# arun-sub/genomicsbench

Measured on AMD Instinct MI355X. Metric: bsw_large_gcups, higher is better.
Workload: dtype int32

## Files before the change

genomicsbench_amd/csrc/bsw_kernels.hip:

```cpp
#include "gbx_internal.h"
#include <atomic>
#include <climits>
#include <cstdlib>

namespace gbx {
namespace {

constexpr int NEG = -(1 << 29);
constexpr int BIGJ = 1 << 20;

constexpr int NCLS = 21;
constexpr int CLS_LDS = NCLS - 1;
constexpr int NTB = 32;
constexpr int NBIN = NCLS * NTB;
constexpr int HDR = 1024;
constexpr int REG_SCORE_LIMIT = 1 << 20;

struct BswDev {
    int o_del, e_del, o_ins, e_ins, oe_del, oe_ins, zdrop, end_bonus, w, max_mat;
    uint32_t colword[5];
    int32_t col4[5];
    uint32_t row0[5];
    uint32_t row1[5];
    uint8_t remap[24];
    uint32_t lrow[5];
    int lane_on;
};

struct BswPairs {
    const uint8_t *ref, *qer;
    const int64_t *idr, *idq;
    const int32_t *len1, *len2, *h0;
    gbx_bsw_result *out;
    int packed = 0;
};

constexpr int WS_HDR = 4 * HDR;
struct BswWork {
    int32_t *counts, *cursors, *base, *bad, *order, *wband;
    int32_t *lbase, *lrank, *lorder, *lchunk;
};

__host__ __device__ inline int cls_of(int qlen, int bound)
{
    if (qlen > 1024 || bound >= REG_SCORE_LIMIT) return CLS_LDS;
    if (qlen > 256) return 19;
    if (qlen <= 128) return (qlen - 1) >> 3;
    return qlen <= 160 ? 16 : qlen <= 192 ? 17 : 18;
}
constexpr int LANE_QMAX = 159;
constexpr int LANE_ROWS = 2 * (LANE_QMAX + 1);
constexpr int LANE_BINS = LANE_ROWS * 256;
constexpr int LANE_SCORE_LIMIT = 8192;
constexpr int LANE_COMPACT_LIMIT = 256;
constexpr int LANE_NRANGE = 5;
constexpr int LANE_RANGE_HI[2][LANE_NRANGE] = {{47, 79, 99, 135, LANE_QMAX}, {39, 79, 103, 127, LANE_QMAX}};
__host__ __device__ inline bool lane_ok(int lane_on, int qlen, int tlen, int h0, int max_mat)
{
    return lane_on && qlen >= 1 && qlen <= LANE_QMAX && tlen >= 1 && h0 >= 0 && h0 + qlen * (max_mat > 0 ? max_mat : 0) < LANE_SCORE_LIMIT;
}
__host__ __device__ inline int lane_key(int qlen, int h0, int max_mat)
{
    const int wide = h0 + qlen * (max_mat > 0 ? max_mat : 0) < LANE_COMPACT_LIMIT ? 0 : 1;
    return ((wide * (LANE_QMAX + 1) + qlen) << 8) | (h0 < 255 ? h0 : 255);
}

__host__ __device__ inline int bin_of(int cls, int tlen)
{
    const int tb = tlen >> 4;
    return cls * NTB + (NTB - 1 - (tb < NTB - 1 ? tb : NTB - 1));
}

__device__ inline int imax3(int a, int b, int c) { return max(max(a, b), c); }

template <int CTRL, int ROWMASK = 0xf, int BANKMASK = 0xf>
__device__ inline int dpp(int old, int x)
{
    return __builtin_amdgcn_update_dpp(old, x, CTRL, ROWMASK, BANKMASK, false);
}
// ... 479 lines not shown
            "v_max3_u32 %[key], %[kin], %[ka], %[kb]\n"
            "v_lshl_or_b32 %[wn], %[v], 16, %[u]\n"
            : [sa] "=&v"(sa), [ta] "=&v"(ta), [tb] "=&v"(tb), [ma] "=&v"(ma), [mb] "=&v"(mb), [x] "=&v"(x), [ha] "=&v"(ha),
              [hb] "=&v"(hb), [td] "=&v"(td), [ed] "=&v"(ed), [ena] "=&v"(ena), [enb] "=&v"(enb), [fd] "=&v"(fd), [ka] "=&v"(ka),
              [kb] "=&v"(kb), [u] "=&v"(u), [v] "=&v"(v), [wn] "=&v"(wn), [f] "+v"(f), [key] "=v"(kout)
            : [w] "v"(w), [qq] "v"(qq), [rw] "v"(rw), [rwn] "v"(rwn), [left] "v"(left), [kin] "v"(kin), [pa] "v"(pa), [pa1] "v"(pa1), [zero] "v"(zero), [oed] "s"(oe_del),
              [edel] "s"(e_del), [eins] "s"(e_ins)
            : "vcc");
    } else {
        int sa, ta, tb, ma, mb, x, ha, td, ti, ed, ena, enb, fd, ka, kb, u, v;
        asm volatile(
            "v_perm_b32 %[sa], %[rwn], %[rw], %[qq]\n"
            "v_cmp_ne_u32_sdwa vcc, %[w], %[zero] src0_sel:BYTE_1 src1_sel:DWORD\n"
            "v_subrev_u32 %[fd], %[eins], %[f]\n"
            "v_add_u32_sdwa %[ta], sext(%[sa]), %[w] dst_sel:DWORD dst_unused:UNUSED_PAD src0_sel:BYTE_0 src1_sel:BYTE_1\n"
            "v_cndmask_b32 %[ma], 0, %[ta], vcc\n"
            "v_cmp_ne_u32_sdwa vcc, %[w], %[zero] src0_sel:BYTE_3 src1_sel:DWORD\n"
            "v_max_i32_sdwa %[x], %[ma], %[w] dst_sel:DWORD dst_unused:UNUSED_PAD src0_sel:DWORD src1_sel:BYTE_0\n"
            "v_add_u32_sdwa %[tb], sext(%[sa]), %[w] dst_sel:DWORD dst_unused:UNUSED_PAD src0_sel:BYTE_1 src1_sel:BYTE_3\n"
            "v_max_i32 %[ha], %[x], %[f]\n"
            "v_subrev_u32 %[td], %[oed], %[ma]\n"
            "v_subrev_u32 %[ti], %[oei], %[ma]\n"
            "v_cndmask_b32 %[mb], 0, %[tb], vcc\n"
            "v_sub_u32_sdwa %[ed], %[w], %[edel] dst_sel:DWORD dst_unused:UNUSED_PAD src0_sel:BYTE_0 src1_sel:DWORD\n"
            "v_max3_i32 %[f], %[fd], %[ti], 0\n"
            "v_max3_i32 %[ena], %[ed], %[td], 0\n"
            "v_max_i32_sdwa %[x], %[mb], %[w] dst_sel:DWORD dst_unused:UNUSED_PAD src0_sel:DWORD src1_sel:BYTE_2\n"
            "v_lshl_or_b32 %[ka], %[ha], 18, %[pa]\n"
            "v_max_i32 %[hb], %[x], %[f]\n"
            "v_subrev_u32 %[td], %[oed], %[mb]\n"
            "v_subrev_u32 %[ti], %[oei], %[mb]\n"
            "v_subrev_u32 %[fd], %[eins], %[f]\n"
            "v_sub_u32_sdwa %[ed], %[w], %[edel] dst_sel:DWORD dst_unused:UNUSED_PAD src0_sel:BYTE_2 src1_sel:DWORD\n"
            "v_max3_i32 %[f], %[fd], %[ti], 0\n"
            "v_max3_i32 %[enb], %[ed], %[td], 0\n"
            "v_lshl_or_b32 %[kb], %[hb], 18, %[pa1]\n"
            "v_lshl_or_b32 %[u], %[left], 8, %[ena]\n"
            "v_lshl_or_b32 %[v], %[ha], 8, %[enb]\n"
            "v_max3_u32 %[key], %[kin], %[ka], %[kb]\n"
            "v_lshl_or_b32 %[wn], %[v], 16, %[u]\n"
            : [sa] "=&v"(sa), [ta] "=&v"(ta), [tb] "=&v"(tb), [ma] "=&v"(ma), [mb] "=&v"(mb), [x] "=&v"(x), [ha] "=&v"(ha),
              [hb] "=&v"(hb), [td] "=&v"(td), [ti] "=&v"(ti), [ed] "=&v"(ed), [ena] "=&v"(ena), [enb] "=&v"(enb), [fd] "=&v"(fd), [ka] "=&v"(ka),
              [kb] "=&v"(kb), [u] "=&v"(u), [v] "=&v"(v), [wn] "=&v"(wn), [f] "+v"(f), [key] "=v"(kout)
            : [w] "v"(w), [qq] "v"(qq), [rw] "v"(rw), [rwn] "v"(rwn), [left] "v"(left), [kin] "v"(kin), [pa] "v"(pa), [pa1] "v"(pa1), [zero] "v"(zero), [oed] "s"(oe_del),
              [oei] "s"(oe_ins), [edel] "s"(e_del), [eins] "s"(e_ins)
            : "vcc");
    }
    left = hb;
    key = kout;
    return wn;
}

#ifdef GBX_BSW_LANE_STATS
__device__ unsigned long long g_bsw_lane_stats[16][4];
#endif
template <bool SYM, bool COMPACT, bool CODE4 = false, bool PACKED = false>
__global__ void __launch_bounds__(64) bsw_lane_kernel(BswDev prm, BswPairs P, BswWork W, int rlo, int rhi, int cols, int slot)
{
    extern __shared__ uint32_t lcell[];
#ifdef GBX_BSW_LANE_STATS
    __shared__ int st_rowmax[2048];
    for (int k = threadIdx.x; k < 2048; k += 64) st_rowmax[k] = 0;
    unsigned long long st_cells = 0, st_rows = 0, st_wcells = 0, st_wrows = 0;
#endif
#define LCELL(byte_addr) (*(uint32_t *)((char *)lcell + (byte_addr)))
#define LCELL16(byte_addr) (*(uint16_t *)((char *)lcell + (byte_addr)))
#define LQ8(byte_addr) (*((uint8_t *)lcell + (byte_addr)))
    const int lane = threadIdx.x;
    const int first = W.lbase[rlo << 8], count = W.lbase[(rhi + 1) << 8] - first;
    const int nchunks = (count + 63) >> 6;
    const int32_t *order = W.lorder + first;
    const int e_ins = prm.e_ins, e_del = prm.e_del, oe_ins = prm.oe_ins, oe_del = prm.oe_del;
    const int cb = lane * 4;
    constexpr int QROW = CODE4 ? 64 : 128;
    const int qb = (cols >> 1) * 256 + (CODE4 ? lane : (lane & 31) * 4 + (lane >> 5) * 2);
    auto LQREAD = [&](int a) -> uint32_t { return CODE4 ? (uint32_t)LQ8(a) : (uint32_t)LCELL16(a); };
    auto QSEL = [](uint32_t q) -> uint32_t { return CODE4 ? (((q >> 4) << 8) | (q & 15u)) : q; };
    auto QLOW = [](uint32_t q) -> uint32_t { return CODE4 ? (q & 15u) : (q & 0xffu); };
    auto cell_at = [&](int j) { return COMPACT ? (j >> 1) * 256 + cb + (j & 1) * 2 : j * 256 + cb; };
    const int tab = COMPACT ? (cols >> 1) * (256 + QROW) + 512 : (cols + 2) * 256 - 128;
    if (lane < 5) *(uint4 *)((char *)lcell + tab + lane * 16) = make_uint4(prm.row0[lane], prm.row1[lane], prm.lrow[lane], 0u);
#define LTAB(base_code) (*(const uint4 *)((const char *)lcell + tab + min((int)(base_code), 4) * 16))
    int rel0 = 0, rel1 = 2, rel2 = 256, rel3 = 258, rel4 = 512, rel5 = 514, rel6 = 768, rel7 = 770;
    asm volatile("" : "+v"(rel0), "+v"(rel1), "+v"(rel2), "+v"(rel3), "+v"(rel4), "+v"(rel5), "+v"(rel6), "+v"(rel7));
    for (;;) {
        int c = 0;
        if (lane == 0) c = atomicAdd(&W.lchunk[slot], 1);
        c = __builtin_amdgcn_readfirstlane(c);
        if (c >= nchunks) break;
        const int hi_ = count - (c << 6), idx = hi_ - 64 + lane;
        const bool have = idx >= 0;
        const int pair = order[have ? idx : 0];
        const int qlen = P.len2[pair], tlen = P.len1[pair], h0 = P.h0[pair];
        const int64_t qo = P.idq[pair], to = P.idr[pair];
        const uint8_t *q = P.qer + (PACKED ? 0 : qo);
        const uint8_t *t = P.ref + (PACKED ? 0 : to);
        auto qpiece = [&](int j) -> uint4 {
            uint4 r;
            if (!PACKED) { __builtin_memcpy(&r, q + j, 16); return r; }
            const int64_t o = qo + j;
            const uint8_t *b = q + (o >> 1);
            uint64_t v;
            __builtin_memcpy(&v, b, 8);
            if (o & 1) v = (v >> 4) | ((uint64_t)b[8] << 60);
            auto spread = [](unsigned h) -> unsigned { return (h & 0xfu) | ((h & 0xf0u) << 4) | ((h & 0xf00u) << 8) | ((h & 0xf000u) << 12); };
            const unsigned lo = (unsigned)v, hi = (unsigned)(v >> 32);
            r.x = spread(lo & 0xffffu); r.y = spread(lo >> 16); r.z = spread(hi & 0xffffu); r.w = spread(hi >> 16);
            return r;
        };
        auto tbase = [&](int i) -> int {
            if (!PACKED) return t[i];
            const int64_t o = to + i;
            return (t[o >> 1] >> ((int)(o & 1) * 4)) & 15;
        };
        {
            uint4 wq = qpiece(0);
            int hrun = h0 - oe_ins + e_ins;
            for (int j0 = 0; j0 <= qlen; j0 += 16) {
                const uint4 cur = wq;
                if (j0 + 16 <= qlen) wq = qpiece(j0 + 16);
                const uint32_t ww[4] = {cur.x, cur.y, cur.z, cur.w};
#pragma unroll
                for (int c = 0; c < 16; c += 2) {
                    const int j = j0 + c;
                    if (j <= qlen) {
                        const uint32_t two = (ww[c >> 2] >> ((c & 3) * 8)) & 0xffffu;
                        const int c0 = j < qlen ? min((int)(two & 0xffu), 4) : 0, c1 = j + 1 < qlen ? min((int)(two >> 8), 4) : 0;
                        const int hv0 = j == 0 ? h0 : max(hrun, 0), hv1 = max(hrun - e_ins, 0);
                        hrun -= 2 * e_ins;
                        if (COMPACT) {
                            LCELL((j >> 1) * 256 + cb) = ((uint32_t)hv0 << 8) | ((uint32_t)hv1 << 24);
                            if (CODE4) LQ8(qb + (j >> 1) * QROW) = (uint8_t)(c0 | (c1 << 4));
                            else LCELL16(qb + (j >> 1) * QROW) = (uint16_t)(c0 | (c1 << 8));
                        } else {
                            LCELL(cell_at(j)) = ((uint32_t)hv0 << 18) | (uint32_t)(c0 * 6);
                            if (j + 1 <= qlen) LCELL(cell_at(j + 1)) = ((uint32_t)hv1 << 18) | (uint32_t)(c1 * 6);
                        }
                    }
                }
            }
        }
        const int w = band_width(prm, qlen);
// ... 96 lines not shown
                left = (int)(left18 >> 18);
                LCELL(abend) = left18 | (LCELL(abend) & 31u);
            }
            const int jfin = beg < end ? end : beg;
            if (jfin == qlen) {
                if (!(g_score > left)) g_i = i;
                g_score = max(g_score, left);
            }
            const int row_best = (int)(key >> 18);
            const int karg = (int)(key & 0x3ffffu) - cb;
            const int row_arg = COMPACT ? ((karg >> 8) << 1) | ((karg >> 1) & 1) : karg >> 8;
            if (row_best == 0) break;
            if (row_best > best) {
                best = row_best; best_i = i; best_j = row_arg;
                off = max(off, abs(row_arg - i));
            } else if (prm.zdrop > 0) {
                const int di = i - best_i, dj = row_arg - best_j;
                if (di > dj) { if (best - row_best - (di - dj) * e_del > prm.zdrop) break; }
                else if (best - row_best - (dj - di) * e_ins > prm.zdrop) break;
            }
            int j = beg;
            if (COMPACT) {
                int k = (sb1 >> 16) ? 3 : 4;
                k = (sb1 & 0xffffu) ? 2 : k;
                k = (sb0 >> 16) ? 1 : k;
                k = (sb0 & 0xffffu) && !(beg & 1) ? 0 : k;
                j = 2 * sp0 + k;
                if (k == 4) while (j < end && LCELL16(cell_at(j)) == 0) ++j;
                j = min(j, end);
                const int nbeg = beg < end ? j : beg;
                const int khi = end - 2 * sq;
                k = (se0 & 0xffffu) ? 0 : -1;
                k = (se0 >> 16) && khi >= 1 ? 1 : k;
                k = (se1 & 0xffffu) && khi >= 2 ? 2 : k;
                k = (se1 >> 16) && khi >= 3 ? 3 : k;
                j = 2 * sq + k;
                if (k < 0 && 2 * sq > nbeg) while (j >= nbeg && LCELL16(cell_at(j)) == 0) --j;
                j = max(j, nbeg - 1);
                j = nbeg > end ? end : j;
                beg = nbeg;
            } else {
                while (j < end && LCELL(cell_at(j)) < 32u) ++j;
                beg = j;
                j = end;
                while (j >= beg && LCELL(cell_at(j)) < 32u) --j;
            }
            end = min(j + 2, qlen);
        }
        gbx_bsw_result r;
        r.score = best; r.tle = best_i + 1; r.gtle = g_i + 1; r.qle = best_j + 1; r.gscore = g_score; r.max_off = off;
        if (have) P.out[pair] = r;
#ifdef GBX_BSW_LANE_STATS
        __builtin_amdgcn_s_waitcnt(0);
        for (int k = threadIdx.x; k < 2048; k += 64) { const int m = st_rowmax[k]; if (m) { st_wcells += 64ull * (unsigned)(m - 1); st_wrows += 64; } st_rowmax[k] = 0; }
#endif
    }
#ifdef GBX_BSW_LANE_STATS
    atomicAdd(&g_bsw_lane_stats[slot][0], st_cells); atomicAdd(&g_bsw_lane_stats[slot][1], st_wcells);
    atomicAdd(&g_bsw_lane_stats[slot][2], st_rows); atomicAdd(&g_bsw_lane_stats[slot][3], st_wrows);
#endif
#undef LCELL
#undef LCELL16
#undef LQ8
#undef LTAB
}


#define GBX_REG_STEP_HEAD(SEL0, SEL1)                                                                                                   \
    "v_cmp_ne_u32_sdwa vcc, %[w], %[zero] src0_sel:BYTE_1 src1_sel:DWORD\n"                                                            \
    "v_subrev_u32 %[fd], %[eins], %[f]\n"                                                                                               \
    "v_add_u32_sdwa %[ta], sext(%[sa]), %[w] dst_sel:DWORD dst_unused:UNUSED_PAD src0_sel:" SEL0 " src1_sel:BYTE_1\n"                  \
    "v_cndmask_b32 %[ma], 0, %[ta], vcc\n"                                                                                              \
    "v_cmp_ne_u32_sdwa vcc, %[w], %[zero] src0_sel:BYTE_3 src1_sel:DWORD\n"                                                            \
    "v_max_i32_sdwa %[x], %[ma], %[w] dst_sel:DWORD dst_unused:UNUSED_PAD src0_sel:DWORD src1_sel:BYTE_0\n"                            \
    "v_add_u32_sdwa %[tb], sext(%[sa]), %[w] dst_sel:DWORD dst_unused:UNUSED_PAD src0_sel:" SEL1 " src1_sel:BYTE_3\n"                  \
    "v_max_i32 %[ha], %[x], %[f]\n"
#define GBX_REG_STEP_SYM(SEL0, SEL1)                                                                                                    \
    GBX_REG_STEP_HEAD(SEL0, SEL1)                                                                                                       \
    "v_subrev_u32 %[td], %[oed], %[ma]\n"                                                                                               \
    "v_cndmask_b32 %[mb], 0, %[tb], vcc\n"                                                                                              \
    "v_sub_u32_sdwa %[ed], %[w], %[edel] dst_sel:DWORD dst_unused:UNUSED_PAD src0_sel:BYTE_0 src1_sel:DWORD\n"                         \
    "v_max3_i32 %[f], %[fd], %[td], 0\n"                                                                                                \
    "v_max3_i32 %[ena], %[ed], %[td], 0\n"                                                                                              \
    "v_max_i32_sdwa %[x], %[mb], %[w] dst_sel:DWORD dst_unused:UNUSED_PAD src0_sel:DWORD src1_sel:BYTE_2\n"                            \
    "v_lshl_or_b32 %[ka], %[ha], 18, %[pa]\n"                                                                                           \
    "v_max_i32 %[hb], %[x], %[f]\n"                                                                                                     \
    "v_subrev_u32 %[td], %[oed], %[mb]\n"                                                                                               \
    "v_subrev_u32 %[fd], %[eins], %[f]\n"                                                                                               \
    "v_sub_u32_sdwa %[ed], %[w], %[edel] dst_sel:DWORD dst_unused:UNUSED_PAD src0_sel:BYTE_2 src1_sel:DWORD\n"                         \
    "v_max3_i32 %[f], %[fd], %[td], 0\n"                                                                                                \
    "v_max3_i32 %[enb], %[ed], %[td], 0\n"                                                                                              \
    "v_lshl_or_b32 %[kb], %[hb], 18, %[pa1]\n"                                                                                          \
    "v_lshl_or_b32 %[u], %[left], 8, %[ena]\n"                                                                                          \
    "v_lshl_or_b32 %[v], %[ha], 8, %[enb]\n"                                                                                            \
    "v_max3_u32 %[key], %[kin], %[ka], %[kb]\n"                                                                                         \
    "v_lshl_or_b32 %[wn], %[v], 16, %[u]\n"
#define GBX_REG_STEP_ASYM(SEL0, SEL1)                                                                                                   \
    GBX_REG_STEP_HEAD(SEL0, SEL1)                                                                                                       \
    "v_subrev_u32 %[td], %[oed], %[ma]\n"                                                                                               \
    "v_subrev_u32 %[ti], %[oei], %[ma]\n"                                                                                               \
    "v_cndmask_b32 %[mb], 0, %[tb], vcc\n"                                                                                              \
    "v_sub_u32_sdwa %[ed], %[w], %[edel] dst_sel:DWORD dst_unused:UNUSED_PAD src0_sel:BYTE_0 src1_sel:DWORD\n"                         \
    "v_max3_i32 %[f], %[fd], %[ti], 0\n"                                                                                                \
    "v_max3_i32 %[ena], %[ed], %[td], 0\n"                                                                                              \
    "v_max_i32_sdwa %[x], %[mb], %[w] dst_sel:DWORD dst_unused:UNUSED_PAD src0_sel:DWORD src1_sel:BYTE_2\n"                            \
    "v_lshl_or_b32 %[ka], %[ha], 18, %[pa]\n"                                                                                           \
    "v_max_i32 %[hb], %[x], %[f]\n"                                                                                                     \
    "v_subrev_u32 %[td], %[oed], %[mb]\n"                                                                                               \
    "v_subrev_u32 %[ti], %[oei], %[mb]\n"                                                                                               \
    "v_subrev_u32 %[fd], %[eins], %[f]\n"                                                                                               \
    "v_sub_u32_sdwa %[ed], %[w], %[edel] dst_sel:DWORD dst_unused:UNUSED_PAD src0_sel:BYTE_2 src1_sel:DWORD\n"                         \
    "v_max3_i32 %[f], %[fd], %[ti], 0\n"                                                                                                \
// ... 45 lines not shown
}
__device__ inline uint32_t bits_from(int lo)
{
    return lo <= 0 ? ~0u : lo >= 32 ? 0u : ~0u << lo;
}
__device__ inline uint32_t bit_span(int lo, int hi)
{
    return lo > hi ? 0u : (hi >= 31 ? ~0u : (2u << hi) - 1u) & ~((1u << lo) - 1u);
}

template <bool SYM, bool HI, int PA>
__device__ __forceinline__ void reg_pair_masked(uint32_t &cell, uint32_t sa, int beg, int end, int &f, int &left, uint32_t &key,
                                                int zero, int oe_del, int oe_ins, int e_del, int e_ins)
{
    constexpr int c0 = PA;
    if (c0 + 1 < end && c0 + 1 >= beg) {
        const uint32_t win = c0 < beg ? cell & 0xffff0000u : cell;
        cell = reg_pair_step<SYM, HI, PA>(win, sa, f, left, key, zero, oe_del, oe_ins, e_del, e_ins);
    } else if (c0 + 1 == end) {
        if (c0 >= beg) {
            const int sc = (int)(int8_t)(sa >> (HI ? 16 : 0));
            const int diag = (int)((cell >> 8) & 0xffu), e = (int)(cell & 0xffu);
            const int m = diag ? diag + sc : 0;
            const int h = imax3(m, e, f);
            key = max(key, ((uint32_t)h << 18) | (uint32_t)PA);
            const int en = imax3(e - e_del, m - oe_del, 0);
            cell = ((uint32_t)h << 24) | ((uint32_t)left << 8) | (uint32_t)en;
            left = h;
        } else {
            cell = (cell & 0xffffu) | ((uint32_t)left << 24);
        }
    } else if (c0 == end) {
        cell = (cell & 0xffff0000u) | ((uint32_t)left << 8);
    }
}

template <bool SYM, int QHI>
__global__ void __launch_bounds__(64, 3) bsw_lane_reg_kernel(BswDev prm, BswPairs P, BswWork W, int rlo, int rhi, int slot)
{
    constexpr int NCP = QHI / 2 + 1;
    constexpr int NB = (NCP + 3) / 4;
    constexpr int NQ = (NCP + 1) / 2;
    constexpr int NW = (2 * NCP + 31) / 32;
    static_assert(NB <= 31, "block masks are 32-bit");
    constexpr int OUT = 1 << 12;
    __shared__ uint2 s_tab[5];
    const int lane = threadIdx.x;
    if (lane < 5) s_tab[lane] = make_uint2(prm.row0[lane], prm.row1[lane]);
    __syncthreads();
    const int first = W.lbase[rlo << 8], count = W.lbase[(rhi + 1) << 8] - first;
    const int nchunks = (count + 63) >> 6;
    const int32_t *order = W.lorder + first;
    const int e_ins = prm.e_ins, e_del = prm.e_del, oe_ins = prm.oe_ins, oe_del = prm.oe_del;
    for (;;) {
        int c = 0;
        if (lane == 0) c = atomicAdd(&W.lchunk[slot], 1);
        c = __builtin_amdgcn_readfirstlane(c);
        if (c >= nchunks) break;
        const int hi_ = count - (c << 6), idx = hi_ - 64 + lane;
        const bool have = idx >= 0;
        const int pair = order[have ? idx : 0];
        const int qlen = P.len2[pair], tlen = P.len1[pair], h0 = P.h0[pair];
        const uint8_t *q = P.qer + P.idq[pair];
        const uint8_t *t = P.ref + P.idr[pair];

        uint32_t qs[NQ];
#pragma unroll
        for (int k = 0; k < (4 * NQ + 15) / 16; ++k) {
            uint4 v = make_uint4(0u, 0u, 0u, 0u);
            if (16 * k <= qlen) __builtin_memcpy(&v, q + 16 * k, 16);
            const uint32_t vv[4] = {v.x, v.y, v.z, v.w};
#pragma unroll
            for (int m = 0; m < 4 && 4 * k + m < NQ; ++m) {
                const uint32_t x = vv[m];
                const uint32_t ge5 = ((((x | 0x80808080u) - 0x05050505u) | x) & 0x80808080u) >> 7;
                const uint32_t msk = ge5 * 0xffu;
                qs[4 * k + m] = (x & ~msk) | (0x04040404u & msk);
            }
        }
        uint32_t cell[NCP];
        {
            int hr = h0 - oe_ins, rem = qlen;
#pragma unroll
            for (int p = 0; p < NCP; ++p) {
                const int hv0 = p == 0 ? h0 : max(hr + e_ins, 0), hv1 = max(hr, 0);
                cell[p] = (rem >= 0 ? (uint32_t)hv0 << 8 : 0u) | (rem >= 1 ? (uint32_t)hv1 << 24 : 0u);
                hr -= 2 * e_ins;
                rem -= 2;
            }
        }
        const int w = band_width(prm, qlen);
        int best = h0, best_i = -1, best_j = -1, g_i = -1, g_score = -1, off = 0;
        int beg = 0, end = qlen;
        bool running = true;
        uint2 mrow = s_tab[min((int)t[0], 4)], mnext = s_tab[min((int)t[1], 4)];
        int tb2 = t[2];
        const uint8_t *tp = t + 3;
        int hrow = h0 - prm.o_del - e_del;
        int imw = -w, ipw = w + 1;
        for (int i = 0;; ++i) {
            if (!__any(running)) break;
            const uint32_t rw = mrow.x, rwn = mrow.y;
            mrow = mnext;
            mnext = s_tab[min(tb2, 4)];
            tb2 = running ? (int)*tp : 0;
            tp += running ? 1 : 0;
            beg = max(beg, imw);
            end = min(min(end, ipw), qlen);
            ++imw; ++ipw;
            int left = beg == 0 ? max(hrow, 0) : 0;
            hrow -= e_del;
// ... 64 lines not shown
                if (!stop) {
                    int k = (sb1 >> 16) ? 3 : 4;
                    k = (sb1 & 0xffffu) ? 2 : k;
                    k = (sb0 >> 16) ? 1 : k;
                    k = (sb0 & 0xffffu) && !(beg & 1) ? 0 : k;
                    int j = 2 * sp0 + k;
                    const int khi = end - 2 * sq;
                    int ke = (se0 & 0xffffu) ? 0 : -1;
                    ke = (se0 >> 16) && khi >= 1 ? 1 : ke;
                    ke = (se1 & 0xffffu) && khi >= 2 ? 2 : ke;
                    ke = (se1 >> 16) && khi >= 3 ? 3 : ke;
                    uint32_t nz[NW];
                    if (k == 4 || ke < 0) {
#pragma unroll
                        for (int u = 0; u < NW; ++u) nz[u] = 0u;
#pragma unroll
                        for (int p = 0; p < NCP; ++p) {
                            const uint32_t two = ((cell[p] & 0xffffu) ? 1u : 0u) | ((cell[p] >> 16) ? 2u : 0u);
                            nz[p >> 4] |= two << ((2 * p) & 31);
                        }
                    }
                    if (k == 4) {
                        int jn = end;
#pragma unroll
                        for (int u = NW - 1; u >= 0; --u) {
                            const uint32_t m = nz[u] & bits_from(j - 32 * u) & ~bits_from(end - 32 * u);
                            jn = m ? 32 * u + __builtin_ctz(m) : jn;
                        }
                        j = jn;
                    }
                    j = min(j, end);
                    const int nbeg = beg < end ? j : beg;
                    j = 2 * sq + ke;
                    if (ke < 0 && 2 * sq > nbeg) {
                        int jl = nbeg - 1;
#pragma unroll
                        for (int u = 0; u < NW; ++u) {
                            const uint32_t m = nz[u] & bits_from(nbeg - 32 * u) & ~bits_from(j + 1 - 32 * u);
                            jl = m ? 32 * u + 31 - __builtin_clz(m) : jl;
                        }
                        j = jl;
                    }
                    j = max(j, nbeg - 1);
                    j = nbeg > end ? end : j;
                    beg = nbeg;
                    end = min(j + 2, qlen);
                }
                running = !stop && i + 1 < tlen;
            }
        }
        gbx_bsw_result r;
        r.score = best; r.tle = best_i + 1; r.gtle = g_i + 1; r.qle = best_j + 1; r.gscore = g_score; r.max_off = off;
        if (have) P.out[pair] = r;
    }
}

typedef void (*RowsFn)(BswDev, BswPairs, BswWork, int);
struct RowKernel { int lpp, cpl; RowsFn fn[2]; std::atomic<int> bpc[2]; const char *name; };
#define GBX_ROW_KERNEL(L, C) { L, C, { bsw_rows_kernel<L, C, false>, bsw_rows_kernel<L, C, true> }, { 0, 0 }, "bsw_rows_" #L "x" #C }
RowKernel row_kernels[] = {
    GBX_ROW_KERNEL(2, 4),  GBX_ROW_KERNEL(2, 8),  GBX_ROW_KERNEL(2, 12), GBX_ROW_KERNEL(2, 16), GBX_ROW_KERNEL(2, 20), GBX_ROW_KERNEL(2, 24),
    GBX_ROW_KERNEL(4, 14), GBX_ROW_KERNEL(4, 16), GBX_ROW_KERNEL(4, 18), GBX_ROW_KERNEL(4, 20), GBX_ROW_KERNEL(4, 22), GBX_ROW_KERNEL(4, 24),
    GBX_ROW_KERNEL(8, 13), GBX_ROW_KERNEL(8, 14), GBX_ROW_KERNEL(8, 15), GBX_ROW_KERNEL(8, 16),
    GBX_ROW_KERNEL(16, 10), GBX_ROW_KERNEL(16, 12), GBX_ROW_KERNEL(16, 16), GBX_ROW_KERNEL(64, 16),
    GBX_ROW_KERNEL(16, 8), GBX_ROW_KERNEL(64, 3), GBX_ROW_KERNEL(64, 4),
};
#undef GBX_ROW_KERNEL
static_assert(sizeof(row_kernels) / sizeof(row_kernels[0]) >= NCLS - 1, "one row kernel per register class");

constexpr uint8_t CLASS_REMAP[3][NCLS] = {
    {0, 1, 2, 3, 4, 5, 6, 7, 8, 9, 10, 11, 12, 13, 14, 15, 16, 17, 18, 19, 20},
    {3, 3, 3, 3, 7, 7, 7, 7, 11, 11, 11, 11, 15, 15, 15, 15, 18, 18, 18, 19, 20},
    {15, 15, 15, 15, 15, 15, 15, 15, 15, 15, 15, 15, 15, 15, 15, 15, 18, 18, 18, 19, 20},
};
int class_mode_for(int64_t n)
{
    const char *e = getenv("GBX_BSW_CLASSMODE");
    if (e && *e >= '0' && *e <= '2') return *e - '0';
    return n < 32768 ? 2 : n < 250000 ? 1 : 0;
}

RowKernel *find_row_kernel(int lpp, int cpl)
{
    for (RowKernel &k : row_kernels)
        if (k.lpp == lpp && k.cpl == cpl) return &k;
    return nullptr;
}

typedef void (*LaneFn)(BswDev, BswPairs, BswWork, int, int, int, int);
enum { LANE_COMPACT = 0, LANE_COMPACT4 = 1, LANE_WIDE = 2 };
#define GBX_LANE_KERNEL(COMPACT, CODE4, PACKED) { bsw_lane_kernel<false, COMPACT, CODE4, PACKED>, bsw_lane_kernel<true, COMPACT, CODE4, PACKED> }
const LaneFn lane_kernels[2][3][2] = {
    { GBX_LANE_KERNEL(true, false, false), GBX_LANE_KERNEL(true, true, false), GBX_LANE_KERNEL(false, false, false) },
    { GBX_LANE_KERNEL(true, false, true),  GBX_LANE_KERNEL(true, true, true),  GBX_LANE_KERNEL(false, false, true) },
};
#undef GBX_LANE_KERNEL

int resident_blocks(std::atomic<int> &cache, const void *fn, int threads, int fallback, int cap)
{
    int bpc = cache.load(std::memory_order_relaxed);
    if (bpc) return bpc;
    if (hipOccupancyMaxActiveBlocksPerMultiprocessor(&bpc, fn, threads, 0) != hipSuccess || bpc < 1) { (void)hipGetLastError(); bpc = fallback; }
    bpc = bpc > cap ? cap : bpc;
    cache.store(bpc, std::memory_order_relaxed);
    return bpc;
}

bool switched_off(const char *name) { const char *e = getenv(name); return e && atoi(e) == 0; }

int make_dev_params(const gbx_bsw_params *p, BswDev *d)
{
    if (p->e_del < 1 || p->e_ins < 1 || p->o_del < 0 || p->o_ins < 0 || p->e_del > 4096 || p->e_ins > 4096 ||
        p->o_del > (1 << 16) || p->o_ins > (1 << 16) || p->w < 0) {
        set_error("bsw: gap penalties must satisfy 0<=o<=65536, 1<=e<=4096, w>=0");
        return GBX_ERR_ARG;
    }
    d->o_del = p->o_del; d->e_del = p->e_del; d->o_ins = p->o_ins; d->e_ins = p->e_ins;
    d->oe_del = p->o_del + p->e_del; d->oe_ins = p->o_ins + p->e_ins;
    d->zdrop = p->zdrop; d->end_bonus = p->end_bonus; d->w = p->w;
    int mx = 0;
    for (int k = 0; k < 25; ++k) mx = p->mat[k] > mx ? p->mat[k] : mx;
    d->max_mat = mx;
    for (int q = 0; q < 5; ++q) {
        uint32_t wv = 0;
        for (int t = 0; t < 4; ++t) wv |= (uint32_t)(uint8_t)p->mat[t * 5 + q] << (8 * t);
        d->colword[q] = wv;
        d->col4[q] = p->mat[4 * 5 + q];
    }
    for (int t = 0; t < 5; ++t) {
        uint32_t wv = 0;
        for (int q = 0; q < 4; ++q) wv |= (uint32_t)(uint8_t)p->mat[t * 5 + q] << (8 * q);
        d->row0[t] = wv;
        d->row1[t] = (uint32_t)(uint8_t)p->mat[t * 5 + 4];
    }
    d->lane_on = 0;
    bool fits6 = true;
    for (int k = 0; k < 25; ++k) fits6 = fits6 && p->mat[k] >= -32 && p->mat[k] <= 31;
    for (int t = 0; t < 5; ++t) {
        uint32_t wv = 0;
        for (int q = 0; q < 5; ++q) wv |= ((uint32_t)p->mat[t * 5 + q] & 63u) << (6 * q);
        d->lrow[t] = wv;
    }
    if (fits6 && p->o_del + p->e_del < LANE_SCORE_LIMIT && p->o_ins + p->e_ins < LANE_SCORE_LIMIT) d->lane_on = -1;
    return GBX_OK;
}

}

constexpr int64_t WS_LANE = (int64_t)(LANE_BINS + 64) + 64;
size_t bsw_workspace_bytes(int64_t n)
{
    return (size_t)(WS_HDR + 4 * (n > 0 ? n : 0) + WS_LANE) * sizeof(int32_t);
}

constexpr int UNPACK_ROUNDS = 4;
__device__ inline unsigned spread4(unsigned h) { return (h & 0xfu) | ((h & 0xf0u) << 4) | ((h & 0xf00u) << 8) | ((h & 0xf000u) << 12); }
__global__ void __launch_bounds__(256) bsw_unpack4_kernel(const uint8_t *__restrict__ packed, uint8_t *__restrict__ out, int64_t lo, int64_t hi)
{
    const int64_t base = lo + (int64_t)blockIdx.x * (256 * 16 * UNPACK_ROUNDS) + threadIdx.x * 16;
    const bool aligned = (((uintptr_t)(packed + (base >> 1)) & 7) == 0) && (((uintptr_t)(out + base) & 15) == 0);
    if (aligned && base + (int64_t)(UNPACK_ROUNDS - 1) * 4096 + 16 <= hi) {
        uint2 v[UNPACK_ROUNDS];
#pragma unroll
        for (int r = 0; r < UNPACK_ROUNDS; ++r) v[r] = *(const uint2 *)(packed + ((base + r * 4096) >> 1));
#pragma unroll
        for (int r = 0; r < UNPACK_ROUNDS; ++r) {
            uint4 q;
            q.x = spread4(v[r].x & 0xffffu); q.y = spread4(v[r].x >> 16); q.z = spread4(v[r].y & 0xffffu); q.w = spread4(v[r].y >> 16);
            *(uint4 *)(out + base + r * 4096) = q;
        }
        return;
    }
    for (int r = 0; r < UNPACK_ROUNDS; ++r) {
        const int64_t o = base + r * 4096;
        if (o >= hi) return;
        if (aligned && o + 16 <= hi) {
            const uint2 v = *(const uint2 *)(packed + (o >> 1));
            uint4 q;
            q.x = spread4(v.x & 0xffffu); q.y = spread4(v.x >> 16); q.z = spread4(v.y & 0xffffu); q.w = spread4(v.y >> 16);
            *(uint4 *)(out + o) = q;
        } else {
            for (int64_t k = o; k < o + 16 && k < hi; ++k) out[k] = (uint8_t)((packed[k >> 1] >> ((k & 1) * 4)) & 0xf);
        }
    }
}

int bsw_unpack4(const uint8_t *d_packed, uint8_t *d_out, int64_t lo, int64_t hi, hipStream_t s)
{
// ... 113 lines not shown
    if (c.dev.lane_on) {
        hipStream_t so;
        if (c.ahead) {
            so = ss->pre[1];
            GBX_HIP(hipMemsetAsync(c.W.lbase, 0, (size_t)WS_LANE * sizeof(int32_t), so));
        } else {
            GBX_HIP(hipMemsetAsync(c.W.lbase, 0, (size_t)WS_LANE * sizeof(int32_t), c.s));
            if ((rc = ss->fork(c.s))) return rc;
            so = ss->side[SideStreams::N - 1];
        }
        Stage st("bsw_lane_sort", so);
        const int sblocks = (int)((n + 255) / 256);
        hipLaunchKernelGGL(bsw_lane_sort_kernel, dim3(sblocks), dim3(256), 0, so, c.dev, c.P, n, c.W, 0);
        hipLaunchKernelGGL(bsw_lane_scan_kernel, dim3(1), dim3(1024), 0, so, c.W);
        hipLaunchKernelGGL(bsw_lane_sort_kernel, dim3(sblocks), dim3(256), 0, so, c.dev, c.P, n, c.W, 1);
        GBX_HIP(hipEventRecord(c.ev_aux, so));
    }
    const int cblocks = (int)((n + CLS_THREADS - 1) / CLS_THREADS);
    {
        Stage st("bsw_classify", c.s_cls);
        hipLaunchKernelGGL(bsw_classify_kernel, dim3(cblocks), dim3(CLS_THREADS), 0, c.s_cls, c.dev, c.P, n, c.W, 0);
        hipLaunchKernelGGL(bsw_scan_kernel, dim3(1), dim3(HDR), 0, c.s_cls, c.W);
        hipLaunchKernelGGL(bsw_classify_kernel, dim3(cblocks), dim3(CLS_THREADS), 0, c.s_cls, c.dev, c.P, n, c.W, 1);
    }
    if (c.ahead) GBX_HIP(hipEventRecord(c.ev_pre, c.s_cls));
    GBX_HIP(hipGetLastError());
    return GBX_OK;
}

static int kernel_streams_wait(const BswCall &c, hipEvent_t ev, int n_side = SideStreams::N)
{
    GBX_HIP(hipStreamWaitEvent(c.s, ev, 0));
    for (int k = 0; k < n_side; ++k) GBX_HIP(hipStreamWaitEvent(c.ss->side[k], ev, 0));
    return GBX_OK;
}

static void launch_row_classes(BswCall &c)
{
    const int nk = c.join_events ? 3 : 4;
    int launched = 0;
    for (int cls = 0; cls < NCLS - 1; ++cls) {
        if (CLASS_REMAP[c.mode][cls] != cls) continue;
        const int sk = (c.mode ? launched++ : cls) % nk;
        hipStream_t sc = c.dev.lane_on || sk == 0 ? c.s : c.ss->side[sk - 1];
        RowKernel &k = row_kernels[cls];
        const int bpc = resident_blocks(k.bpc[c.sym], (const void *)k.fn[c.sym], 256, 2, 8);
        const int gpb = 256 / k.lpp;
        const int64_t want = (c.n + gpb - 1) / gpb, cap = (int64_t)c.cus * bpc;
        Stage st(k.name, sc);
        hipLaunchKernelGGL(k.fn[c.sym], dim3((int)(want < cap ? want : cap)), dim3(256), 0, sc, c.dev, c.P, c.W, cls);
    }
}

static void launch_lane_reg(const BswCall &c, hipStream_t sc, int64_t want, int rlo, int rhi, int slot)
{
    static_assert(LANE_RANGE_HI[0][2] == 99, "bsw_lane_reg_kernel instance");
    typedef void (*LaneRegFn)(BswDev, BswPairs, BswWork, int, int, int);
    static const LaneRegFn reg_fn[2] = {bsw_lane_reg_kernel<false, 99>, bsw_lane_reg_kernel<true, 99>};
    static std::atomic<int> reg_bpc[2];
    const int64_t cap = (int64_t)c.cus * resident_blocks(reg_bpc[c.sym], (const void *)reg_fn[c.sym], 64, 8, INT_MAX);
    hipLaunchKernelGGL(reg_fn[c.sym], dim3((unsigned)(want < cap ? want : cap)), dim3(64), 0, sc, c.dev, c.P, c.W, rlo, rhi, slot);
    g_lane_reg_launches.fetch_add(1, std::memory_order_relaxed);
}

static void launch_lanes(const BswCall &c)
{
    static const char *names[2][LANE_NRANGE] = {{"bsw_lane_c47", "bsw_lane_c79", "bsw_lane_c99", "bsw_lane_c135", "bsw_lane_c159"},
                                                {"bsw_lane_w39", "bsw_lane_w79", "bsw_lane_w103", "bsw_lane_w127", "bsw_lane_w159"}};
    const int64_t want = (c.n + 63) / 64;
    for (int fmt = 1; fmt >= 0; --fmt) {
        for (int r = LANE_NRANGE - 1; r >= 0; --r) {
            const int qlo = r ? LANE_RANGE_HI[fmt][r - 1] + 1 : 1, qhi = LANE_RANGE_HI[fmt][r];
            const int cols = (qhi + 3) & ~1;
            const int kind = fmt ? LANE_WIDE : qhi > 99 ? LANE_COMPACT4 : LANE_COMPACT;
            const size_t lds = fmt ? (size_t)(cols + 2) * 256 : (size_t)(cols / 2) * (kind == LANE_COMPACT4 ? 320 : 384) + 640;
            const int fit = (int)((size_t)160 * 1024 / lds), per_cu = fit > 16 ? 16 : fit;
            const int sk = (LANE_NRANGE - 1 - r) & 3;
            hipStream_t sc = sk == 0 ? c.s : c.ss->side[sk - 1];
            const int64_t cap = (int64_t)c.cus * per_cu;
            const int rlo = fmt * (LANE_QMAX + 1) + qlo, rhi = fmt * (LANE_QMAX + 1) + qhi, slot = fmt * LANE_NRANGE + r;
            Stage st(names[fmt][r], sc);
            if (fmt == 0 && !c.P.packed && qhi == 99 && !switched_off("GBX_BSW_LANE_REG")) { launch_lane_reg(c, sc, want, rlo, rhi, slot); continue; }
            hipLaunchKernelGGL(lane_kernels[c.P.packed][kind][c.sym], dim3((unsigned)(want < cap ? want : cap)), dim3(64), lds, sc,
                               c.dev, c.P, c.W, rlo, rhi, cols, slot);
        }
    }
}

static int launch_lds(const BswCall &c)
{
    const size_t lds_bytes = (size_t)(GBX_BSW_MAX_QLEN + 1) * 2 * sizeof(int);
    static std::atomic<uint64_t> attr_set[2];
    int cur = 0;
    GBX_HIP(hipGetDevice(&cur));
    const uint64_t bit = (uint64_t)1 << (cur & 63);
    if (cur >= 128 || !(attr_set[cur >> 6].load(std::memory_order_acquire) & bit)) {
        GBX_HIP(hipFuncSetAttribute((const void *)bsw_lds_kernel, hipFuncAttributeMaxDynamicSharedMemorySize, (int)lds_bytes));
        if (cur < 128) attr_set[cur >> 6].fetch_or(bit, std::memory_order_release);
    }
    const int blocks = (int)(c.n < (int64_t)c.cus * 2 ? c.n : (int64_t)c.cus * 2);
    Stage st("bsw_lds", c.s);
    hipLaunchKernelGGL(bsw_lds_kernel, dim3(blocks), dim3(64), lds_bytes, c.s, c.dev, c.P, c.W, CLS_LDS);
    return GBX_OK;
}

int bsw_launch(const gbx_bsw_params *p, int64_t n,
               const uint8_t *d_ref, const uint8_t *d_qer,
               const int64_t *d_idr, const int64_t *d_idq,
               const int32_t *d_len1, const int32_t *d_len2, const int32_t *d_h0,
               gbx_bsw_result *d_out, void *d_work, size_t work_bytes, hipStream_t s, hipEvent_t *join_events,
               const BswChunkPrep *prep)
{
    if (n == 0) return GBX_OK;
    if (n > 0x7fffffffLL - 1024) { set_error("bsw: more than 2^31 pairs in one call"); return GBX_ERR_UNSUPPORTED; }
    if (work_bytes < bsw_workspace_bytes(n)) { set_error("bsw: workspace too small"); return GBX_ERR_ARG; }
    BswCall c;
    int rc = make_dev_params(p, &c.dev);
    if (rc) return rc;
    c.n = n; c.mode = class_mode_for(n); c.cus = 256;
    for (int k = 0; k < NCLS; ++k) c.dev.remap[k] = CLASS_REMAP[c.mode][k];
    c.P = {d_ref, d_qer, d_idr, d_idq, d_len1, d_len2, d_h0, d_out};
    int32_t *wi = (int32_t *)d_work, *wl = wi + WS_HDR + 4 * n;
    c.W = {wi, wi + HDR, wi + 2 * HDR, wi + 3 * HDR, wi + WS_HDR, wi + WS_HDR + n, wl, wi + WS_HDR + 3 * n, wi + WS_HDR + 2 * n, wl + LANE_BINS + 64};
    c.dev.lane_on = c.dev.lane_on && lane_wanted(n) ? 1 : 0;
    c.sym = c.dev.oe_ins == c.dev.oe_del;
    c.s = s; c.join_events = join_events; c.prep = prep;
    if ((rc = side_streams(&c.ss))) return rc;
    std::unique_lock<std::mutex> side_lock(c.ss->mu);
    if ((rc = plan_call(c))) return rc;
    if (c.phase != 2) {
        if ((rc = queue_prepare(c))) return rc;
        if (c.phase == 1) return GBX_OK;
    }
    if (c.ahead) {
        if ((rc = kernel_streams_wait(c, c.ev_pre))) return rc;
        if (c.phase == 2 && (rc = kernel_streams_wait(c, prep->uploaded))) return rc;
    }
    int dev_id = 0;
    (void)hipGetDevice(&dev_id);
    (void)hipDeviceGetAttribute(&c.cus, hipDeviceAttributeMultiprocessorCount, dev_id);
    if (!c.dev.lane_on && !c.ahead && (rc = c.ss->fork(s))) return rc;
    if (!c.no_rows) launch_row_classes(c);
    if (c.dev.lane_on) {
        if ((rc = kernel_streams_wait(c, c.ev_aux, c.ahead ? SideStreams::N : SideStreams::N - 1))) return rc;
        launch_lanes(c);
    }
    if (!join_events && (rc = c.ss->join(s))) return rc;
    if (!c.no_rows && (rc = launch_lds(c))) return rc;
    if (join_events) {
        GBX_HIP(hipEventRecord(join_events[0], s));
        for (int k = 0; k < SideStreams::N; ++k) GBX_HIP(hipEventRecord(join_events[1 + k], c.ss->side[k]));
    }
    GBX_HIP(hipGetLastError());
    return GBX_OK;
}

}

extern "C" long long gbx_debug_bsw_lane_reg_launches(void)
{
    return gbx::g_lane_reg_launches.load(std::memory_order_relaxed);
}

#ifdef GBX_BSW_LANE_STATS
extern "C" int gbx_debug_bsw_lane_stats(unsigned long long *out, int reset)
{
    if (hipMemcpyFromSymbol(out, HIP_SYMBOL(gbx::g_bsw_lane_stats), sizeof(unsigned long long) * 64) != hipSuccess) return -1;
    if (reset) { unsigned long long z[64] = {0}; if (hipMemcpyToSymbol(HIP_SYMBOL(gbx::g_bsw_lane_stats), z, sizeof(z)) != hipSuccess) return -1; }
    return 0;
}
#endif
```

Baseline: 2532.

## Prioritize large-LDS lane waves and cap register-kernel residency per CU

Adds s_setprio(3) for LDS-heavy lane kernel waves (LDS footprint of at least 20KB) and priority 0 for the register-resident lane kernel, so that co-resident long-row waves are favoured in scheduling. The grid size of the register lane kernel is also capped using VGPR counts, leaving register room for two LDS lane waves per SIMD, with an env override. The aim is to balance the concurrent kernels running on side streams so the long-tail LDS classes finish sooner. It also adds optional timing stats under a debug macro. The risk is that the register kernel gets fewer resident waves and less throughput.

```diff
diff --git a/genomicsbench_amd/csrc/bsw_kernels.hip b/genomicsbench_amd/csrc/bsw_kernels.hip
--- a/genomicsbench_amd/csrc/bsw_kernels.hip
+++ b/genomicsbench_amd/csrc/bsw_kernels.hip
@@ -25,6 +25,7 @@
     uint8_t remap[24];
     uint32_t lrow[5];
     int lane_on;
+    int lane_prio;
 };
 
 struct BswPairs {
@@ -610,8 +611,17 @@
 }
 
 #ifdef GBX_BSW_LANE_STATS
-__device__ unsigned long long g_bsw_lane_stats[16][4];
+constexpr int LANE_NSTAT = 6;
+__device__ unsigned long long g_bsw_lane_stats[16][LANE_NSTAT];
 #endif
+__host__ __device__ constexpr int lane_lds_bytes(bool compact, bool code4, int cols)
+{
+    return compact ? (cols / 2) * (code4 ? 320 : 384) + 640 : (cols + 2) * 256;
+}
+__host__ __device__ constexpr int lane_wave_prio(int on, int lds_bytes)
+{
+    return on && lds_bytes >= 20 * 1024 ? 3 : 0;
+}
 template <bool SYM, bool COMPACT, bool CODE4 = false, bool PACKED = false>
 __global__ void __launch_bounds__(64) bsw_lane_kernel(BswDev prm, BswPairs P, BswWork W, int rlo, int rhi, int cols, int slot)
 {
@@ -619,7 +629,7 @@
 #ifdef GBX_BSW_LANE_STATS
     __shared__ int st_rowmax[2048];
     for (int k = threadIdx.x; k < 2048; k += 64) st_rowmax[k] = 0;
-    unsigned long long st_cells = 0, st_rows = 0, st_wcells = 0, st_wrows = 0;
+    unsigned long long st_cells = 0, st_rows = 0, st_wcells = 0, st_wrows = 0, st_chunks = 0, st_ticks = 0;
 #endif
 #define LCELL(byte_addr) (*(uint32_t *)((char *)lcell + (byte_addr)))
 #define LCELL16(byte_addr) (*(uint16_t *)((char *)lcell + (byte_addr)))
@@ -641,11 +651,15 @@
 #define LTAB(base_code) (*(const uint4 *)((const char *)lcell + tab + min((int)(base_code), 4) * 16))
     int rel0 = 0, rel1 = 2, rel2 = 256, rel3 = 258, rel4 = 512, rel5 = 514, rel6 = 768, rel7 = 770;
     asm volatile("" : "+v"(rel0), "+v"(rel1), "+v"(rel2), "+v"(rel3), "+v"(rel4), "+v"(rel5), "+v"(rel6), "+v"(rel7));
+    if (lane_wave_prio(prm.lane_prio, lane_lds_bytes(COMPACT, CODE4, cols)) == 3) __builtin_amdgcn_s_setprio(3);
     for (;;) {
         int c = 0;
         if (lane == 0) c = atomicAdd(&W.lchunk[slot], 1);
         c = __builtin_amdgcn_readfirstlane(c);
         if (c >= nchunks) break;
+#ifdef GBX_BSW_LANE_STATS
+        const unsigned long long st_t0 = wall_clock64();
+#endif
         const int hi_ = count - (c << 6), idx = hi_ - 64 + lane;
         const bool have = idx >= 0;
         const int pair = order[have ? idx : 0];
@@ -848,12 +862,14 @@
         if (have) P.out[pair] = r;
 #ifdef GBX_BSW_LANE_STATS
         __builtin_amdgcn_s_waitcnt(0);
+        st_chunks += 1; st_ticks += wall_clock64() - st_t0;
         for (int k = threadIdx.x; k < 2048; k += 64) { const int m = st_rowmax[k]; if (m) { st_wcells += 64ull * (unsigned)(m - 1); st_wrows += 64; } st_rowmax[k] = 0; }
 #endif
     }
 #ifdef GBX_BSW_LANE_STATS
     atomicAdd(&g_bsw_lane_stats[slot][0], st_cells); atomicAdd(&g_bsw_lane_stats[slot][1], st_wcells);
     atomicAdd(&g_bsw_lane_stats[slot][2], st_rows); atomicAdd(&g_bsw_lane_stats[slot][3], st_wrows);
+    if (lane == 0) { atomicAdd(&g_bsw_lane_stats[slot][4], st_chunks); atomicAdd(&g_bsw_lane_stats[slot][5], st_ticks); }
 #endif
 #undef LCELL
 #undef LCELL16
@@ -1005,11 +1021,18 @@
     const int nchunks = (count + 63) >> 6;
     const int32_t *order = W.lorder + first;
     const int e_ins = prm.e_ins, e_del = prm.e_del, oe_ins = prm.oe_ins, oe_del = prm.oe_del;
+#ifdef GBX_BSW_LANE_STATS
+    unsigned long long st_chunks = 0, st_ticks = 0;
+#endif
+    __builtin_amdgcn_s_setprio(0);
     for (;;) {
         int c = 0;
         if (lane == 0) c = atomicAdd(&W.lchunk[slot], 1);
         c = __builtin_amdgcn_readfirstlane(c);
         if (c >= nchunks) break;
+#ifdef GBX_BSW_LANE_STATS
+        const unsigned long long st_t0 = wall_clock64();
+#endif
         const int hi_ = count - (c << 6), idx = hi_ - 64 + lane;
         const bool have = idx >= 0;
         const int pair = order[have ? idx : 0];
@@ -1180,7 +1203,14 @@
         gbx_bsw_result r;
         r.score = best; r.tle = best_i + 1; r.gtle = g_i + 1; r.qle = best_j + 1; r.gscore = g_score; r.max_off = off;
         if (have) P.out[pair] = r;
-    }
+#ifdef GBX_BSW_LANE_STATS
+        __builtin_amdgcn_s_waitcnt(0);
+        st_chunks += 1; st_ticks += wall_clock64() - st_t0;
+#endif
+    }
+#ifdef GBX_BSW_LANE_STATS
+    if (lane == 0) { atomicAdd(&g_bsw_lane_stats[slot][4], st_chunks); atomicAdd(&g_bsw_lane_stats[slot][5], st_ticks); }
+#endif
 }
 
 typedef void (*RowsFn)(BswDev, BswPairs, BswWork, int);
@@ -1262,6 +1292,7 @@
         d->row1[t] = (uint32_t)(uint8_t)p->mat[t * 5 + 4];
     }
     d->lane_on = 0;
+    d->lane_prio = 0;
     bool fits6 = true;
     for (int k = 0; k < 25; ++k) fits6 = fits6 && p->mat[k] >= -32 && p->mat[k] <= 31;
     for (int t = 0; t < 5; ++t) {
@@ -1481,13 +1512,33 @@
     }
 }
 
+static int wave_vgprs(const void *fn)
+{
+    hipFuncAttributes a;
+    if (hipFuncGetAttributes(&a, fn) != hipSuccess) { (void)hipGetLastError(); return 0; }
+    return a.numRegs >= 1 && a.numRegs <= 512 ? (a.numRegs + 7) & ~7 : 0;
+}
+
+static std::atomic<int> g_lane_reg_waves{0};
+
 static void launch_lane_reg(const BswCall &c, hipStream_t sc, int64_t want, int rlo, int rhi, int slot)
 {
     static_assert(LANE_RANGE_HI[0][2] == 99, "bsw_lane_reg_kernel instance");
     typedef void (*LaneRegFn)(BswDev, BswPairs, BswWork, int, int, int);
     static const LaneRegFn reg_fn[2] = {bsw_lane_reg_kernel<false, 99>, bsw_lane_reg_kernel<true, 99>};
-    static std::atomic<int> reg_bpc[2];
-    const int64_t cap = (int64_t)c.cus * resident_blocks(reg_bpc[c.sym], (const void *)reg_fn[c.sym], 64, 8, INT_MAX);
+    static std::atomic<int> reg_bpc[2], reg_plan[2];
+    const int resident = resident_blocks(reg_bpc[c.sym], (const void *)reg_fn[c.sym], 64, 8, INT_MAX);
+    int plan = reg_plan[c.sym].load(std::memory_order_relaxed);
+    if (!plan) {
+        const int rv = wave_vgprs((const void *)reg_fn[c.sym]), lv = wave_vgprs((const void *)lane_kernels[0][LANE_COMPACT4][c.sym]);
+        plan = rv && lv && 512 - 2 * lv >= rv ? 4 * ((512 - 2 * lv) / rv) : resident;
+        reg_plan[c.sym].store(plan, std::memory_order_relaxed);
+    }
+    int per_cu = plan;
+    if (const char *e = getenv("GBX_BSW_LANE_REG_WAVES")) { const int v = atoi(e); if (v >= 1) per_cu = v; }
+    per_cu = per_cu < resident ? per_cu : resident;
+    g_lane_reg_waves.store(per_cu, std::memory_order_relaxed);
+    const int64_t cap = (int64_t)c.cus * per_cu;
     hipLaunchKernelGGL(reg_fn[c.sym], dim3((unsigned)(want < cap ? want : cap)), dim3(64), 0, sc, c.dev, c.P, c.W, rlo, rhi, slot);
     g_lane_reg_launches.fetch_add(1, std::memory_order_relaxed);
 }
@@ -1502,7 +1553,7 @@
             const int qlo = r ? LANE_RANGE_HI[fmt][r - 1] + 1 : 1, qhi = LANE_RANGE_HI[fmt][r];
             const int cols = (qhi + 3) & ~1;
             const int kind = fmt ? LANE_WIDE : qhi > 99 ? LANE_COMPACT4 : LANE_COMPACT;
-            const size_t lds = fmt ? (size_t)(cols + 2) * 256 : (size_t)(cols / 2) * (kind == LANE_COMPACT4 ? 320 : 384) + 640;
+            const size_t lds = (size_t)lane_lds_bytes(!fmt, kind == LANE_COMPACT4, cols);
             const int fit = (int)((size_t)160 * 1024 / lds), per_cu = fit > 16 ? 16 : fit;
             const int sk = (LANE_NRANGE - 1 - r) & 3;
             hipStream_t sc = sk == 0 ? c.s : c.ss->side[sk - 1];
@@ -1552,6 +1603,7 @@
     int32_t *wi = (int32_t *)d_work, *wl = wi + WS_HDR + 4 * n;
     c.W = {wi, wi + HDR, wi + 2 * HDR, wi + 3 * HDR, wi + WS_HDR, wi + WS_HDR + n, wl, wi + WS_HDR + 3 * n, wi + WS_HDR + 2 * n, wl + LANE_BINS + 64};
     c.dev.lane_on = c.dev.lane_on && lane_wanted(n) ? 1 : 0;
+    c.dev.lane_prio = switched_off("GBX_BSW_LANE_PRIO") ? 0 : 1;
     c.sym = c.dev.oe_ins == c.dev.oe_del;
     c.s = s; c.join_events = join_events; c.prep = prep;
     if ((rc = side_streams(&c.ss))) return rc;
@@ -1591,11 +1643,16 @@
     return gbx::g_lane_reg_launches.load(std::memory_order_relaxed);
 }
 
+extern "C" int gbx_debug_bsw_lane_reg_waves(void)
+{
+    return gbx::g_lane_reg_waves.load(std::memory_order_relaxed);
+}
+
 #ifdef GBX_BSW_LANE_STATS
 extern "C" int gbx_debug_bsw_lane_stats(unsigned long long *out, int reset)
 {
-    if (hipMemcpyFromSymbol(out, HIP_SYMBOL(gbx::g_bsw_lane_stats), sizeof(unsigned long long) * 64) != hipSuccess) return -1;
-    if (reset) { unsigned long long z[64] = {0}; if (hipMemcpyToSymbol(HIP_SYMBOL(gbx::g_bsw_lane_stats), z, sizeof(z)) != hipSuccess) return -1; }
+    if (hipMemcpyFromSymbol(out, HIP_SYMBOL(gbx::g_bsw_lane_stats), sizeof(gbx::g_bsw_lane_stats)) != hipSuccess) return -1;
+    if (reset) { unsigned long long z[16 * gbx::LANE_NSTAT] = {0}; if (hipMemcpyToSymbol(HIP_SYMBOL(gbx::g_bsw_lane_stats), z, sizeof(z)) != hipSuccess) return -1; }
     return 0;
 }
 #endif
```

Result: faster. 2602 (median of 6 runs) (+2.8%).
